# yangao07/LAMSA

Hardware: AMD Instinct MI355X
Metric: aligned Gbase/s, 10 kbp ONT-error reads (12%: sub/ins/del 4% each), -T ont2d vs GRCh37-sized stand-in; inputs resident in HBM when the timed region starts (upload excluded: see pcie_inclusive_*) (higher is better)
Workload: dtype int32

## Files before the change

### lamsa_amd/csrc/hp_align_api.hip

```cpp
#include <hip/hip_runtime.h>
#include <algorithm>
#include <atomic>
#include <map>
#include <mutex>
#include <stdlib.h>
#include <string.h>
#include <time.h>
#include "hp_phase.h"
#include "hp_handle.h"
#include "hp_hostprep.h"

using namespace hp;

#ifndef HP_WAVES_PER_SIMD
#define HP_WAVES_PER_SIMD 4
#endif
__global__ __launch_bounds__(64, HP_WAVES_PER_SIMD) void k_align_batch(AlignArgs a)
{
    __shared__ int32_t lds[HP_BOTH_LDS_WORDS];
    const int slot = blockIdx.x;
    for (;;) {
        int u = 0;
        if (wv::leader()) u = atomicAdd(a.counter, 1);
        u = wv::uni(u);
// ... 410 lines not shown
    S->valid = true;
    return LAMSA_HP_OK;
}

static int cap_waves(int n_waves, size_t slab_per_wave, int n_cu)
{
    static const size_t budget = []() { size_t f = 0, t = 0; if (hipMemGetInfo(&f, &t) != hipSuccess || t == 0) { t = (size_t)288 << 30; f = t; } return std::min(t / 4, f / 3); }();
    if (slab_per_wave * (size_t)n_waves <= budget) return n_waves;
    size_t fit = budget / (slab_per_wave ? slab_per_wave : 1);
    if (n_cu > 0 && fit >= (size_t)n_cu) fit -= fit % (size_t)n_cu;
    return fit < 1 ? 1 : (int)fit;
}

#ifdef HP_PROF
static void prof_report(Slot &T, const long long *d_prof, int n)
{
    if (!d_prof) return;
    {
        std::vector<long long> pr((size_t)n * 64);
        hipMemcpy(pr.data(), d_prof, sizeof(long long) * pr.size(), hipMemcpyDeviceToHost);
        if (const char *dump = getenv("LAMSA_HP_PROF_DUMP")) {
            if (FILE *fp = fopen(dump, "wb")) {
                for (int r = 0; r < n; ++r) { long long hl[2] = {T.h_H[r], T.h_len[r]}; fwrite(hl, 8, 2, fp); fwrite(&pr[(size_t)r * 64], 8, 64, fp); }
                fclose(fp);
            }
        }
        std::vector<int> idx((size_t)n); for (int i = 0; i < n; ++i) idx[i] = i;
        auto tot = [&](int r) { long long t = 0; for (int k = 0; k < 6; ++k) t += pr[(size_t)r * 64 + k]; return t; };
        std::sort(idx.begin(), idx.end(), [&](int x, int y) { return tot(x) > tot(y); });
        long long sum[64] = {0}; for (int r = 0; r < n; ++r) for (int k = 0; k < 64; ++k) sum[k] += pr[(size_t)r * 64 + k];
        fprintf(stderr, "[HP_PROF] cycles: setup chain1 fill1 chain2 fill2 publish | in chain1: init+minext mainscan track pop-loop bound+flines | o_l H\n");
        fprintf(stderr, "[HP_PROF] SUM  "); for (int k = 0; k < 11; ++k) fprintf(stderr, " %lld", sum[k] / 1000000); fprintf(stderr, " (Mcycles) targets %lld trips %lld init_Mcyc %lld\n", sum[11], sum[12], sum[13] / 1000000);
#ifdef HP_PROF_TRACK
        fprintf(stderr, "[HP_PROF] branch tracking (-DHP_PROF_TRACK: the line_build stamps below are off): marking pass %lld Mcyc; %lld seeds visited; %lld tracks, %lld Mcyc in them, %lld steps up; "
                        "%lld arrivals at a node with several sons, %lld Mcyc in cut_branch\n", sum[16] / 1000000, sum[19], sum[18], sum[17] / 1000000, sum[20], sum[21], sum[22] / 1000000);
#endif
        fprintf(stderr, "[HP_PROF] line_build: %lld lines (%lld without a gap), %lld anchors, %lld gaps | Mcyc: anchor walk %lld, gap list %lld, gaps in lanes %lld, gaps one by one %lld, assembly %lld\n",
                sum[21], sum[22], sum[12], sum[23], sum[16] / 1000000, sum[17] / 1000000, sum[18] / 1000000, sum[19] / 1000000, sum[20] / 1000000);
        fprintf(stderr, "[HP_PROF] gaps: %lld in lines with fewer than HP_GAP_MIN gaps (%lld lines with gaps); lane gaps: %lld hits scanned, %lld refused (range too long or too many active hits)\n", sum[54], sum[55], sum[11], sum[13]);
        { const char *nm[] = {"ksw_global", "ksw_extend", "backtrack", "ref_fetch", "head_fix", "frag_extend", "split_mapping", "tail_fix", "res_split", "res_aux", "mini_line_regs", "sort index"};
          for (int k = 0; k < 12; ++k) fprintf(stderr, "[HP_PROF] %-16s %8lld Mcyc %10lld calls\n", nm[k], sum[24 + 2 * k] / 1000000, sum[25 + 2 * k]);
#ifdef HP_PROF_FILL
          fprintf(stderr, "[HP_PROF] in frags_merge: boundary repair (merge_cigar_full) %lld Mcyc %lld calls; junctions through split_mapping %lld Mcyc %lld calls; fragments of several seeds %lld Mcyc %lld calls; 64-step gathers %lld Mcyc %lld\n", sum[16] / 1000000, sum[17], sum[18] / 1000000, sum[19], sum[20] / 1000000, sum[21], sum[22] / 1000000, sum[23]);
#endif
          fprintf(stderr, "[HP_PROF] direction-matrix bytes in HBM %lld (%lld jobs); hits passed through nodes_per_init %lld (%lld calls)\n", sum[52], sum[53], sum[54], sum[55]);
          fprintf(stderr, "[HP_PROF] chain_first start: seed loop %lld, node_set loop %lld, min_extend %lld Mcyc (%lld reads with a MIN pass)\n", sum[56] / 1000000, sum[57] / 1000000, sum[58] / 1000000, sum[59]);
          fprintf(stderr, "[HP_PROF] query <= 62: ksw_extend %lld Mcyc %lld calls, ksw_global %lld Mcyc %lld calls\n", sum[60] / 1000000, sum[61], sum[62] / 1000000, sum[63]);
          const char *bn[] = {"[bi_extend total]", "[bi_extend after left ext]", "17-32", "33-64", "65-128", "129-256", "257-512", ">512"};
          for (int k = 0; k < 2; ++k) fprintf(stderr, "[HP_PROF] ksw_extend qlen %-8s %8lld Mcyc %10lld calls\n", bn[k], sum[48 + 2 * k] / 1000000, sum[49 + 2 * k]); }
        {
            std::vector<long long> pd((size_t)n * 64);
            hipMemcpy(pd.data(), d_prof + ((size_t)n + 1) * 64, sizeof(long long) * pd.size(), hipMemcpyDeviceToHost);
            long long sd[64] = {0}; for (int r = 0; r < n; ++r) for (int k = 0; k < 64; ++k) sd[k] += pd[(size_t)r * 64 + k];
            const char *cn[] = {"one set, q <= 62", "packed, one set", "packed, two sets", "band 1 set", "band 2 sets", "band 4 sets", "int32 sets", "LDS / HBM rows"};
            for (int c = 0; c < 8; ++c) fprintf(stderr, "[HP_PROF] wave jobs, ksw_extend %-18s %8lld Mcyc %10lld Mcells %9lld calls %10lld rows\n", cn[c], sd[4 * c] / 1000000, sd[4 * c + 1] / 1000000, sd[4 * c + 2], sd[4 * c + 3]);
        }
        for (int q = 0; q < 8 && q < n; ++q) { int r = idx[q]; fprintf(stderr, "[HP_PROF] read %d L=%d:", r, T.h_len[r]); for (int k = 0; k < 11; ++k) fprintf(stderr, " %lld", pr[(size_t)r * 64 + k] / 1000000); fprintf(stderr, " | o_l %lld H %lld | targets %lld trips %lld init_Mcyc %lld\n", pr[(size_t)r * 64 + 14], pr[(size_t)r * 64 + 15], pr[(size_t)r * 64 + 11], pr[(size_t)r * 64 + 12], pr[(size_t)r * 64 + 13] / 1000000); }
    }
}
#endif

struct PhasedLayout { size_t bytes, o[15]; int unit_cap, lj_cap, wj_cap; int64_t fl_cap, line_cap, job_cap; };
static PhasedLayout phased_layout(int n, int64_t n_hits, int64_t n_bases, int64_t stream_cap)
{
    PhasedLayout Y;
    const size_t n_ent = (size_t)n_hits + (size_t)n + 1;
    Y.unit_cap = 8 * n + 1024;
    Y.fl_cap = 4 * n_hits + 2304 * (int64_t)n + 4096; Y.line_cap = stream_cap + 64 * (int64_t)Y.unit_cap;
    Y.job_cap = std::min<int64_t>(0x7fffff00ll, 4096 + 256 * (int64_t)n + 2 * n_bases);
    Y.lj_cap = (int)std::min<int64_t>(0x3fffffffll, 1024 + 16 * (int64_t)n + n_bases / 100);
    Y.wj_cap = (int)std::min<int64_t>(0x3fffffffll, 1024 + 32 * (int64_t)n + n_bases / 200);
    size_t off = 0;
    auto place = [&](size_t bytes) { size_t o = off; off = al256(off + bytes + 16); return o; };
    const size_t sz[15] = {sizeof(PhaseArgs), sizeof(PhaseCtl), sizeof(RdMeta) * ((size_t)n + 1), sizeof(NodeS) * n_ent, 4 * n_ent, 8 * n_ent, sizeof(UnitRec) * 2 * (size_t)Y.unit_cap,
                           4 * 2 * (size_t)PH_NBUCKET * Y.unit_cap, 4 * (size_t)Y.fl_cap, 4 * (size_t)Y.line_cap, 4 * (size_t)Y.job_cap, sizeof(LjRec) * (size_t)Y.lj_cap, 4 * (size_t)LJ_NBUCKET * Y.lj_cap,
                           sizeof(WjRec) * (size_t)Y.wj_cap, 4 * (size_t)WJ_NBUCKET * Y.wj_cap};
    for (int k = 0; k < 15; ++k) Y.o[k] = place(sz[k]);
    Y.bytes = off;
    return Y;
}
static int64_t main_stream_cap(int n, int64_t n_bases, int tags) { return 1024 + (int64_t)n * 256 + 4 * n_bases + (tags ? (int64_t)n * 128 + 2 * n_bases : 0); }

struct SlabPlan { size_t chain, fill, wj, wjb, wjb_off; int w_chain, w_fill, w_dp, w_wj, n_wjb, shape; size_t bytes; };
static int chain_shape(const lamsa_hp_para &P, int64_t n_reads, int64_t n_bases)
{
    static const int force = getenv("LAMSA_HP_CHAIN_SHAPE") ? atoi(getenv("LAMSA_HP_CHAIN_SHAPE")) : -1;
    if (force >= 0 && force < 3) return force;
    const int64_t mean_L = n_reads > 0 ? n_bases / n_reads : 0, ss = P.seed_step > 0 ? P.seed_step : 1;
    const int64_t est = mean_L / ss * 2 / 3;
    for (int k = 0; k < 2; ++k) if (est <= g_chain_shapes[k].lds_words / 5) return k;
    return 2;
}
static SlabPlan slab_plan(lamsa_hp_handle *h, int max_L, int max_H, bool shared = false, int shape = 0)
{
    SlabPlan Q;
    Q.shape = shape;
    const lamsa_hp_para &P = h->para;
    Q.chain = al256(((size_t)256 << 10) + 128 * (size_t)max_L + 424 * (size_t)max_H);
    Q.fill = al256(((size_t)256 << 10) + (h->result_tags ? 152 : 128) * (size_t)max_L + sizeof(cig_t) * 3 * HP_LJ_CIG * 64 + (size_t)HP_LJ_QSMALL * HP_LJ_TSMALL * 64 + 64);
    { static const int kb = getenv("LAMSA_HP_WJ_SLAB_KB") ? atoi(getenv("LAMSA_HP_WJ_SLAB_KB")) : 0;
      Q.wj = ((size_t)(kb > 0 ? kb : 1024) << 10) + 33 * 256; }
    Q.wjb = al256((size_t)wj_need(&P, WJ_HEAD, max_L, max_L + 2 * P.hash_step + 64) + ((size_t)64 << 10)) + 33 * 256;
    if (Q.wjb < Q.wj) Q.wjb = Q.wj;
    if (g_nowave) Q.fill = std::max(Q.fill, slab_bytes_for(P, max_L, max_H, 1, h->result_tags));
    if (h->scratch_limit) { const size_t lim = al256(h->scratch_limit); Q.chain = std::min(Q.chain, lim); Q.fill = std::min(Q.fill, lim); Q.wj = std::min(Q.wj, lim); Q.wjb = std::min(Q.wjb, lim); }
    int pc = 0, pf = 0, pd = 0, pw = 0;
    if (hipOccupancyMaxActiveBlocksPerMultiprocessor(&pc, g_chain_shapes[shape].k1, 64, 0) != hipSuccess || pc < 1) pc = 4 * g_chain_shapes[shape].waves_per_simd;
    if (hipOccupancyMaxActiveBlocksPerMultiprocessor(&pf, k_fill, 64, 0) != hipSuccess || pf < 1) pf = 4;
// ... 347 lines not shown
```

### lamsa_amd/csrc/hp_ksw.h

```cpp
#pragma once
#include "hp_core.h"

namespace hp {

#define HP_ZSTRIDE(n_col) ((((n_col) + 7) >> 3) << 2)
HP_INL size_t z_cap(const Ctx &cx) { const int w = cx.lds_words - (2 * HP_LDS_CELLS + HP_LDS_CELLS / 4); return w > 0 ? (size_t)w * 4 : 0; }
HP_INL size_t z_cap_pk(const Ctx &cx) { return cx.lds_words > 0 ? (size_t)cx.lds_words * 4 : 0; }
#define HP_ZFITS(n_col, rows) ((size_t)HP_ZSTRIDE(n_col) * (size_t)(rows) <= z_cap(cx))
HP_INL int z_nibble(int dir) { return (dir & 3) | ((dir >> 2) & 1) << 2 | ((dir >> 5) & 1) << 3; }
HP_INL void z_row_clear(HP_L uint8_t *LZ, int row, int n_col) {
    HP_L int *p = (HP_L int *)(LZ + row * HP_ZSTRIDE(n_col));
    const int nd = HP_ZSTRIDE(n_col) >> 2;
    for (int d0 = 0; d0 < nd; d0 += 64) { WAVE_FOR(l) { if (d0 + l < nd) p[d0 + l] = -1; } }
}
HP_INL void z_put(HP_L uint8_t *LZ, int row, int n_col, int c, int dir) {
    HP_L int *p = (HP_L int *)(LZ + row * HP_ZSTRIDE(n_col)) + (c >> 3);
    wv::lds_and(p, (int)~((unsigned)(~z_nibble(dir) & 0xf) << ((c & 7) << 2)));
}

HP_FN void dp_backtrack(Ctx &cx, const HP_L uint8_t *lz, const uint8_t *z, const int32_t *rowb, int n_col, int w, int i, int k, CigV &out, int pk_stride = 0)
{
    pk_stride = wv::uni(pk_stride);
    const bool in_lds = z == nullptr;
    const HP_G uint8_t *gz = (const HP_G uint8_t *)wv::uni64((long long)z);
// ... 763 lines not shown
                    if (j == end) Es[c][l] = 0;
                    nz[l] = j >= beg && j <= end && (Hs[c][l] != 0 || Es[c][l] != 0);
                }
                nzm[c] = wv::ballot(nz);
            }
            const int jj = beg < end ? end : beg;
            if (jj == qlen) {
                max_ie = gscore > h_last ? max_ie : i;
                gscore = gscore > h_last ? gscore : h_last;
            }
            if (mrow == 0) { stop_rows = true; break; }
            if (mrow > max) { max = mrow; max_i = i; max_j = mj; }
            else if (zdrop > 0) {
                if (i - max_i > mj - max_j) { if (max - mrow - ((i - max_i) - (mj - max_j)) * e_del > zdrop) { stop_rows = true; break; } }
                else { if (max - mrow - ((mj - max_j) - (i - max_i)) * e_ins > zdrop) { stop_rows = true; break; } }
            }
            {
                const int e_set = end >> 6;
                const unsigned long long e_bit = 1ull << (end & 63);
                bool end_nz = false, got = false;
                int nb = end, jl = -1;
#pragma unroll
                for (int c = 0; c < NS; ++c) {
                    unsigned long long lo = nzm[c];
                    if (c == e_set) { end_nz = lo & e_bit; lo &= ~e_bit; }
                    if (!got && lo) { nb = 64 * c + __builtin_ctzll(lo); got = true; }
                }
                if (got) {
                    bool gl = false;
#pragma unroll
                    for (int c = NS - 1; c >= 0; --c) if (!gl && nzm[c]) { jl = 64 * c + 63 - __builtin_clzll(nzm[c]); gl = true; }
                } else jl = end_nz ? end : end - 1;
                beg = nb;
                end = jl + 2 < qlen ? jl + 2 : qlen;
            }
        }
    }
    int i, k;
    if (gscore <= 0 || gscore <= max - end_bonus) { i = max_i; k = max_j; }
    else { i = max_ie; k = qlen - 1; }
    er.qle = k + 1; er.tle = i + 1; er.score = max;
    if (out) { wv::sync(); HP_T0(tb0_); dp_backtrack(cx, zl ? LZ : nullptr, z, rowb, n_col, w, i, k, *out); HP_TADD(cx, 28, tb0_); }
    cx.n_cells += cells_;
    arena_release(cx.tmp, mark);
    HP_TADD(cx, 26, te0_);
    return er;
}

#define HP_PK_QMAX(ns) (128 * (ns) - 2)
#ifndef HP_PK_RT
#define HP_PK_RT 1
#endif
#define HP_PK_IDENT (-16000)

HP_INL int pkb_sets_q(int qlen, int w)
{
    for (int ns = 1; ns <= 4; ns *= 2) if (2 * w + 3 + 18 * ns <= 128 * ns || qlen + 3 <= 128 * ns) return ns;
    return 0;
}
HP_INL bool pkb_extend_ok(const lamsa_hp_para *P, int qlen, int h0, int ns)
{
    const int mx = P->match > P->mis ? P->match : P->mis;
    const int pen = (P->ins_ext_o > P->del_ext_o ? P->ins_ext_o : P->del_ext_o) + (P->ins_ext_e > P->del_ext_e ? P->ins_ext_e : P->del_ext_e);
    const int ext = P->ins_ext_e > P->del_ext_e ? P->ins_ext_e : P->del_ext_e;
    return ns > 0 && mx > 0 && mx < 256 && pen >= 0 && pen < 4000 && P->ins_ext_e >= 0 && P->del_ext_e >= 0 && P->ins_ext_o >= 0 && P->del_ext_o >= 0 &&
           (long long)h0 + (long long)qlen * mx < 23000 && (long long)(128 * ns + 2) * ext < 8000 && qlen + 128 * ns < 32000;
}
template <int NS>
HP_NOINL ExtRes ksw_extend_band(Ctx &cx, int qlen, Seq q, int tlen, Seq t, int w, int h0, CigV *out)
{
    long long cells_ = 0;
    ExtRes er; er.score = 0; er.qle = 0; er.tle = 0;
    HP_T0(te0_);
    qlen = wv::uni(qlen); tlen = wv::uni(tlen); w = wv::uni(w); h0 = wv::uni(h0);
    const lamsa_hp_para *P = cx.P;
    const int o_ins = wv::uni(P->ins_ext_o), e_ins = wv::uni(P->ins_ext_e), o_del = wv::uni(P->del_ext_o), e_del = wv::uni(P->del_ext_e);
    const int end_bonus = wv::uni(P->end_bonus), zdrop = wv::uni(P->zdrop);
    const int oe_del = o_del + e_del, oe_ins = o_ins + e_ins;
    const int n_col = qlen < 2 * w + 1 ? qlen : 2 * w + 1;
    constexpr int LC = 2 * NS, WN = 128 * NS, zs = 64 * NS;
    const size_t mark = arena_mark(cx.tmp);
    uint8_t *z = (uint8_t *)arena_alloc(cx, (size_t)zs * tlen + 16);
    int32_t *rowb = (int32_t *)arena_alloc(cx, sizeof(int32_t) * 2 * ((size_t)tlen + 1));
    if (!z || !rowb) { arena_release(cx.tmp, mark); return er; }
#ifdef HP_PROF
    if (cx.prof) { cx.prof[52] += (long long)zs * tlen; cx.prof[53] += 1; }
#endif
    HP_G uint8_t *gz = (HP_G uint8_t *)wv::uni64((long long)z);
    HP_G int32_t *growb = (HP_G int32_t *)wv::uni64((long long)rowb);
    const int sc_match = wv::uni(P->match), sc_mis = -wv::uni(P->mis);
    const HP_G uint8_t *gq = (const HP_G uint8_t *)wv::uni64((long long)q.p); const int qs = wv::uni(q.stride);
    const HP_G uint8_t *gt = (const HP_G uint8_t *)wv::uni64((long long)t.p); const int ts = wv::uni(t.stride);
    const int h1v = h0 > oe_ins ? h0 - oe_ins : 0;
    const int OEI = pk::rep(oe_ins), OED = pk::rep(oe_del), EI = pk::rep(e_ins), ED = pk::rep(e_del);
    const int DSC = pk::rep(sc_match - sc_mis), MIS = pk::rep(sc_mis), IDENT = pk::rep(HP_PK_IDENT);
#define HP_PKB_EH0(j) ((j) == 0 ? h0 : ((j) == 1 ? h1v : (((j) <= qlen && h1v - ((j) - 2) * e_ins > e_ins) ? h1v - ((j) - 1) * e_ins : 0)))
#define HP_PKB_LOAD(jb_) do { \
        _Pragma("unroll") for (int r_ = 0; r_ < NS; ++r_) { \
            int hv_[2], oh_ = 0, nn_ = 0; \
            _Pragma("unroll") for (int b_ = 0; b_ < 2; ++b_) { \
                const int j_ = (jb_) + 2 * r_ + b_; \
                hv_[b_] = HP_PKB_EH0(j_); \
                const int code_ = j_ < qlen ? (int)gq[(long)j_ * qs] : 4; \
                if (code_ < 4) oh_ |= 1 << (code_ + 16 * b_); else nn_ |= (int)(0xffffu << (16 * b_)); \
            } \
            Hs[r_][l] = pk::pack(hv_[0], hv_[1]); Es[r_][l] = 0; qoh[r_][l] = oh_; qN[r_][l] = nn_; \
        } \
        JB[l] = pk::rep(jb_); } while (0)
    wv::Lane<int> Hs[NS], Es[NS], qoh[NS], qN[NS], hcur[NS], M[NS], INB[NS], JRE[NS], pre[NS], JB, tl;
    WAVE_FOR(l) { tl[l] = 4; HP_PKB_LOAD(LC * l); }
    int top = WN;
    int max = h0, max_i = -1, max_j = -1, max_ie = -1, gscore = -1;
    int beg = 0, end = qlen;
    bool stop_rows = false;
    for (int ib = 0; ib < tlen && !stop_rows; ib += 64) {
        { WAVE_FOR(l) { const int ii = ib + l; tl[l] = ii < tlen ? gt[(long)ii * ts] : 4; } }
        const int ti_first = wv::bcast(tl, 0);
        const int ie = ib + 64 < tlen ? ib + 64 : tlen;
        for (int i = ib; i < ie; ++i) {
            const int ti = i == ib ? ti_first : wv::bcast(tl, i & 63);
            if (beg < i - w) beg = i - w;
            if (end > i + w + 1) end = i + w + 1;
            if (end > qlen) end = qlen;
            cells_ += end > beg ? end - beg : 0;
            { WAVE_FOR(l) { if (l < 2) growb[2 * i + l] = l ? end : beg; } }
            int h1_init;
            if (beg == 0) { h1_init = h0 - (o_del + e_del * (i + 1)); if (h1_init < 0) h1_init = 0; }
            else h1_init = 0;
            if (beg >= end) {
                if (beg == qlen) { max_ie = gscore > h1_init ? max_ie : i; gscore = gscore > h1_init ? gscore : h1_init; }
                stop_rows = true; break;
            }
            if (end + 3 > top) {
                const int lr = (top / LC) & 63;
                WAVE_FOR(l) { const int d = (l - lr) & 63; if (d < 8) { const int jb = top + d * LC; HP_PKB_LOAD(jb); } }
                top += 8 * LC;
            }
            const int tsh = ti & 3, tN = ti > 3 ? -1 : 0;
            const int BEG = pk::rep(beg), END = pk::rep(end), H1 = pk::rep(h1_init);
            const int l0 = (beg / LC) & 63;
            wv::Lane<int> ka, kb;
            WAVE_FOR(l) {
                int run = HP_PK_IDENT;
#pragma unroll
                for (int r = 0; r < NS; ++r) {
                    const int jp = pk::add(JB[l], pk::pack(2 * r, 2 * r + 1));
                    const int in = pk::neg_mask(pk::sub(jp, END)) & ~pk::neg_mask(pk::sub(jp, BEG));
                    const int eq = (qoh[r][l] >> tsh) & 0x00010001;
                    const int S = pk::add(pk::mul(eq, DSC), MIS) | qN[r][l] | tN;
                    const int hm = Hs[r][l];
                    const int m = pk::mul(pk::add(hm, S), pk::min_u(hm, 0x00010001));
                    const int t1 = pk::max(pk::sub(m, OEI), 0);
                    const int jre = pk::mul(pk::sub(jp, BEG), EI);
                    const int k = pk::sel(in, pk::add(t1, jre), IDENT);
                    const int klo = pk::lo(k), khi = pk::hi(k);
                    const int p0 = run; run = run > klo ? run : klo;
                    const int p1 = run; run = run > khi ? run : khi;
                    M[r][l] = m; INB[r][l] = in; JRE[r][l] = jre; pre[r][l] = pk::pack(p0, p1);
                }
                ka[l] = l >= l0 ? run : HP_PK_IDENT; kb[l] = l < l0 ? run : HP_PK_IDENT;
            }
            const int topA = wv::scan_max_excl_top(ka, HP_PK_IDENT);
            wv::scan_max_excl(kb, HP_PK_IDENT);
            wv::Lane<int> best;
            WAVE_FOR(l) {
                const int pl = l >= l0 ? ka[l] : (topA > kb[l] ? topA : kb[l]);
                const int PP = pk::rep(pl);
                int zw = 0, bk = -1;
#pragma unroll
                for (int r = 0; r < NS; ++r) {
                    const int jre = JRE[r][l], in = INB[r][l], m = M[r][l];
                    const int pr = pk::max(pre[r][l], PP);
                    int f = pk::max(pk::add(pk::sub(pr, jre), EI), pk::sub(0, jre));
                    const int tI = pk::max(pk::sub(m, OEI), 0);
                    int ee = Es[r][l];
                    const int m1 = pk::neg_mask(pk::sub(ee, m));
                    int h = pk::max(m, ee);
                    const int m2 = pk::neg_mask(pk::sub(f, h));
                    int d = pk::sel(m2, ~m1 & 0x00010001, 0x00020002);
                    h = pk::max(h, f);
                    const int tD = pk::max(pk::sub(m, OED), 0);
                    ee = pk::sub(ee, ED);
                    d |= pk::neg_mask(pk::sub(tD, ee)) & 0x00040004;
                    ee = pk::max(ee, tD);
                    f = pk::sub(f, EI);
                    d |= pk::neg_mask(pk::sub(tI, f)) & 0x00080008;
                    Es[r][l] = pk::sel(in, ee, Es[r][l]);
                    const int hc = pk::sel(in, h, -1);
                    hcur[r][l] = hc;
                    zw |= ((d | (d >> 12)) & 0xff) << (8 * r);
                    const int jp = pk::add(JB[l], pk::pack(2 * r, 2 * r + 1));
                    const int k0 = (int)(((unsigned)hc << 16) | ((unsigned)jp & 0xffffu)), k1 = (int)(((unsigned)hc & 0xffff0000u) | ((unsigned)jp >> 16));
                    bk = bk > k0 ? bk : k0; bk = bk > k1 ? bk : k1;
                }
                best[l] = bk;
                if constexpr (NS == 1) gz[(long)i * zs + l] = (uint8_t)zw;
                else if constexpr (NS == 2) *(HP_G uint16_t *)(gz + (long)i * zs + 2 * l) = (uint16_t)zw;
                else *(HP_G uint32_t *)(gz + (long)i * zs + 4 * l) = (uint32_t)zw;
            }
            int mrow = 0, mj = -1;
            { const int b = wv::reduce_max(best); if (b >= 0) { mrow = b >> 16; mj = b & 0xffff; } }
            int h_last;
            {
                const int le = ((end - 1) / LC) & 63, sl = (end - 1) % LC;
                int v = 0;
#pragma unroll
                for (int r = 0; r < NS; ++r) if ((sl >> 1) == r) v = wv::bcast(hcur[r], le);
                h_last = (sl & 1) ? pk::hi(v) : pk::lo(v);
            }
            wv::Lane<int> rot = hcur[NS - 1], LB;
            wv::ror1(rot);
            WAVE_FOR(l) {
                int bits = 0;
#pragma unroll
                for (int r = 0; r < NS; ++r) {
                    const int below = r > 0 ? hcur[r > 0 ? r - 1 : 0][l] : rot[l];
                    const int hsh = pk::shift_up(hcur[r][l], below);
                    const int in = INB[r][l];
                    const int upd = ~pk::neg_mask(hsh);
                    int hs = Hs[r][l], es = Es[r][l];
                    hs = pk::sel(upd, hsh, hs);
                    hs = pk::sel(in & ~upd, H1, hs);
                    es &= ~(upd & ~in);
                    Hs[r][l] = hs; Es[r][l] = es;
                    const int nzh = pk::min_u((hs | es) & (in | upd), 0x00010001);
                    bits |= ((nzh | (nzh >> 15)) & 3) << (2 * r);
                }
                LB[l] = bits;
            }
            if (end == qlen) {
                max_ie = gscore > h_last ? max_ie : i;
                gscore = gscore > h_last ? gscore : h_last;
            }
            if (mrow == 0) { stop_rows = true; break; }
            if (mrow > max) { max = mrow; max_i = i; max_j = mj; }
            else if (zdrop > 0) {
                if (i - max_i > mj - max_j) { if (max - mrow - ((i - max_i) - (mj - max_j)) * e_del > zdrop) { stop_rows = true; break; } }
                else { if (max - mrow - ((mj - max_j) - (i - max_i)) * e_ins > zdrop) { stop_rows = true; break; } }
            }
            {
                const unsigned long long any = wv::ballot(LB);
                int nb = end, jl = end - 1;
                if (any) {
                    const unsigned long long rt = l0 ? ((any >> l0) | (any << (64 - l0))) : any;
                    const int df = __builtin_ctzll(rt), dl = 63 - __builtin_clzll(rt);
                    const int bf = wv::bcast(LB, (l0 + df) & 63), bl = wv::bcast(LB, (l0 + dl) & 63);
                    const int bb = beg / LC;
                    const int jf = (bb + df) * LC + __builtin_ctz((unsigned)bf), jx = (bb + dl) * LC + (31 - __builtin_clz((unsigned)bl));
                    if (jf < end) nb = jf;
                    jl = jx;
                }
                beg = nb;
                end = jl + 2 < qlen ? jl + 2 : qlen;
            }
        }
    }
#undef HP_PKB_LOAD
#undef HP_PKB_EH0
    int i, k;
    if (gscore <= 0 || gscore <= max - end_bonus) { i = max_i; k = max_j; }
    else { i = max_ie; k = qlen - 1; }
    er.qle = k + 1; er.tle = i + 1; er.score = max;
    if (out) { wv::sync(); HP_T0(tb0_); dp_backtrack(cx, nullptr, z, rowb, n_col, w, i, k, *out, zs); HP_TADD(cx, 28, tb0_); }
    cx.n_cells += cells_;
    arena_release(cx.tmp, mark);
    HP_TADD(cx, 26, te0_);
    return er;
}

#define HP_PKG_NEG (-12000)
#define HP_PKG_IDENT (-24000)
HP_INL bool pk_global_ok(const lamsa_hp_para *P, int qlen, int tlen, int o_del, int e_del, int o_ins, int e_ins)
{
    const int mx = P->match > P->mis ? P->match : P->mis;
    const long long o = o_del > o_ins ? o_del : o_ins, e = e_del > e_ins ? e_del : e_ins;
    return mx > 0 && mx < 256 && o_del >= 0 && e_del >= 0 && o_ins >= 0 && e_ins >= 0 && o + e * ((long long)qlen + tlen + 4) + (long long)mx * (qlen + 2) < 4000;
}
template <int NS>
HP_NOINL int ksw_global_pk(Ctx &cx, int qlen, Seq q, int tlen, Seq t, int o_del, int e_del, int o_ins, int e_ins, int w, CigV *out)
{
    long long cells_ = 0;
    HP_T0(tg0_);
    qlen = wv::uni(qlen); tlen = wv::uni(tlen); w = wv::uni(w);
    o_del = wv::uni(o_del); e_del = wv::uni(e_del); o_ins = wv::uni(o_ins); e_ins = wv::uni(e_ins);
    const int oe_del = o_del + e_del, oe_ins = o_ins + e_ins;
    const int n_col = qlen < 2 * w + 1 ? qlen : 2 * w + 1;
    const int zs = 64 * NS;
    const size_t mark = arena_mark(cx.tmp);
    const bool zl = (size_t)zs * (size_t)tlen <= z_cap_pk(cx);
    if (out && zl) ++cx.lds_epoch;
    uint8_t *z = (out && !zl) ? (uint8_t *)arena_alloc(cx, (size_t)zs * tlen + 1) : nullptr;
    if (out && !zl && !z) { arena_release(cx.tmp, mark); return 0; }
    HP_L uint8_t *LZ = (HP_L uint8_t *)cx.lds;
    HP_G uint8_t *gz = (HP_G uint8_t *)wv::uni64((long long)z);
    const int sc_match = wv::uni(cx.P->match), sc_mis = -wv::uni(cx.P->mis);
    const HP_G uint8_t *gq = (const HP_G uint8_t *)wv::uni64((long long)q.p); const int qs = wv::uni(q.stride);
    const HP_G uint8_t *gt = (const HP_G uint8_t *)wv::uni64((long long)t.p); const int ts = wv::uni(t.stride);
    const int OEI = pk::rep(oe_ins), OED = pk::rep(oe_del), EI = pk::rep(e_ins), ED = pk::rep(e_del);
    const int DSC = pk::rep(sc_match - sc_mis), MIS = pk::rep(sc_mis), IDENT = pk::rep(HP_PKG_IDENT), NEG = pk::rep(HP_PKG_NEG);
    wv::Lane<int> Hs[NS], Es[NS], qoh[NS], qN[NS], hcur[NS], jp0, jep0, tl;
    WAVE_FOR(l) { jp0[l] = pk::pack(2 * l, 2 * l + 1); jep0[l] = pk::pack(2 * l * e_ins, (2 * l + 1) * e_ins); tl[l] = 4; }
#pragma unroll
    for (int c = 0; c < NS; ++c) {
        WAVE_FOR(l) {
            int hv[2], oh = 0, nn = 0;
#pragma unroll
            for (int b = 0; b < 2; ++b) {
                const int j = 128 * c + 2 * l + b;
                hv[b] = j == 0 ? 0 : (j <= w ? -(o_ins + e_ins * j) : HP_PKG_NEG);
                const int code = j < qlen ? (int)gq[(long)j * qs] : 4;
                if (code < 4) oh |= 1 << (code + 16 * b); else nn |= (int)(0xffffu << (16 * b));
            }
            Hs[c][l] = pk::pack(hv[0], hv[1]); Es[c][l] = NEG;
            qoh[c][l] = oh; qN[c][l] = nn;
        }
    }
// ... 239 lines not shown
        if (mrow > max) { max = mrow; max_i = i; max_j = mj; }
        else if (zdrop > 0) {
            if (i - max_i > mj - max_j) { if (max - mrow - ((i - max_i) - (mj - max_j)) * e_del > zdrop) { stop_rows = true; break; } }
            else { if (max - mrow - ((mj - max_j) - (i - max_i)) * e_ins > zdrop) { stop_rows = true; break; } }
        }
        {
            const int nb = first_nz >= 0 ? first_nz : end;
            int jl;
            if (h_last != 0 && end >= nb) jl = end;
            else if (last_nz >= nb && last_nz >= 0) jl = last_nz;
            else jl = nb - 1;
            beg = nb;
            end = jl + 2 < qlen ? jl + 2 : qlen;
        }
    }
    }
#undef HP_EH0
    int i, k;
    if (gscore <= 0 || gscore <= max - end_bonus) { i = max_i; k = max_j; }
    else { i = max_ie; k = qlen - 1; }
    er.qle = k + 1; er.tle = i + 1; er.score = max;
    if (out) { wv::sync(); HP_T0(tb0_); dp_backtrack(cx, zl ? LZ : nullptr, z, rowb, n_col, w, i, k, *out); HP_TADD(cx, 28, tb0_); }
    cx.n_cells += cells_;
    arena_release(cx.tmp, mark);
    HP_TADD(cx, 26, te0_);
    return er;
}

HP_INL int ksw_extend(Ctx &cx, int qlen, Seq q, int tlen, Seq t, int w, int h0, int *qle, int *tle, CigV *out)
{
    if (out) out->n = 0;
    if (qle) *qle = 0;
    if (tle) *tle = 0;
    if (qlen < 0 || tlen < 0 || h0 <= 0) { cx.status |= ST_REFEXIT; return 0; }
    {
        const lamsa_hp_para *P = cx.P;
        int mx = P->match > 0 ? P->match : 0;
        if (-P->mis > mx) mx = -P->mis;
        int max_ins = (int)((double)(qlen * mx + P->end_bonus - P->ins_ext_o) / P->ins_ext_e + 1.);
        max_ins = max_ins > 1 ? max_ins : 1;
        w = w < max_ins ? w : max_ins;
        int max_del = (int)((double)(qlen * mx + P->end_bonus - P->del_ext_o) / P->del_ext_e + 1.);
        max_del = max_del > 1 ? max_del : 1;
        w = w < max_del ? w : max_del;
    }
    const long long cells0_ = cx.n_cells; (void)cells0_;
    ExtRes er;
    int cls_ = 0; (void)cls_;
    HP_T0(tcls_);
    if (qlen <= HP_REG_QMAX) er = ksw_extend_reg(cx, qlen, q, tlen, t, w, h0, out);
    else if (HP_PK_RT && pkb_extend_ok(cx.P, qlen, h0, pkb_sets_q(qlen, w))) {
        HP_STAT(22);
        const int ns = pkb_sets_q(qlen, w);
        cls_ = ns == 1 ? 3 : (ns == 2 ? 4 : 5);
        er = ns == 1 ? ksw_extend_band<1>(cx, qlen, q, tlen, t, w, h0, out) : (ns == 2 ? ksw_extend_band<2>(cx, qlen, q, tlen, t, w, h0, out) : ksw_extend_band<4>(cx, qlen, q, tlen, t, w, h0, out));
    }
    else if (qlen <= HP_REGN_QMAX(2)) { HP_STAT(17); cls_ = 6; er = ksw_extend_regn<2>(cx, qlen, q, tlen, t, w, h0, out); }
    else if (qlen <= HP_REGN_QMAX(3) && HP_REGN_SETS >= 3) { HP_STAT(17); cls_ = 6; er = ksw_extend_regn<3>(cx, qlen, q, tlen, t, w, h0, out); }
    else if (qlen <= HP_REGN_QMAX(4) && HP_REGN_SETS >= 4) { HP_STAT(17); cls_ = 6; er = ksw_extend_regn<4>(cx, qlen, q, tlen, t, w, h0, out); }
    else { cls_ = 7; er = 2 * w + 4 + 64 <= HP_LDS_CELLS ? ksw_extend_lds(cx, qlen, q, tlen, t, w, h0, out) : ksw_extend_wide(cx, qlen, q, tlen, t, w, h0, out); }
#ifdef HP_PROF
    if (cx.prof_dp) { cx.prof_dp[4 * cls_] += wv::clock() - tcls_; cx.prof_dp[4 * cls_ + 1] += cx.n_cells - cells0_; cx.prof_dp[4 * cls_ + 2] += 1; cx.prof_dp[4 * cls_ + 3] += er.tle; }
#endif
    HP_DPLOG(0, qlen, tlen, w, cx.n_cells - cells0_);
    if (qle) *qle = er.qle;
    if (tle) *tle = er.tle;
    return er.score;
}

HP_INL int ksw_extend_c(Ctx &cx, int qlen, Seq q, int tlen, Seq t, int w, int h0, int *qle, int *tle, CigV *out)
{
    ksw_extend(cx, qlen, q, tlen, t, w, h0, qle, tle, out);
    if (*qle == qlen) return 0;
    if (*tle == tlen) return 1;
    return 2;
}
HP_INL int ksw_extend_r(Ctx &cx, int qlen, Seq q, int tlen, Seq t, int w, int h0, int *qre, int *tre, CigV *out)
{
    Seq rq, rt;
    rq.p = q.p + (long)(qlen > 0 ? qlen - 1 : 0) * q.stride; rq.stride = -q.stride;
    rt.p = t.p + (long)(tlen > 0 ? tlen - 1 : 0) * t.stride; rt.stride = -t.stride;
    ksw_extend(cx, qlen, rq, tlen, rt, w, h0, qre, tre, out);
    if (*qre == qlen) return 0;
    if (*tre == tlen) return 1;
    return 2;
}

HP_INL void sw_mid_fix(Ctx &cx, CigV &out, const cig_t *lc, int ln, const cig_t *rc, int rn,
                      int qlen, Seq q, int lqe, int rqe, int tlen, Seq t, int lte, int rte)
{
    const lamsa_hp_para *P = cx.P;
    int Sn = qlen - lqe - rqe, Hn = tlen - lte - rte, half = P->split_len / 2;
    if (iabs(Sn) >= half || iabs(Hn) >= half || iabs(Sn - Hn) >= half || tlen < 0 || qlen < 0) {
        cig_pushv(cx, out, lc, ln);
        cig_push0(cx, out, (cig_t)((uint32_t)Sn << 4) | C_S);
        cig_push0(cx, out, (cig_t)((uint32_t)Hn << 4) | C_H);
        cig_pushv(cx, out, rc, rn);
    } else {
        const size_t mark = arena_mark(cx.tmp);
        CigV g;
        if (cig_alloc(cx, g, qlen + tlen + 2)) {
            ksw_global(cx, qlen, q, tlen, t, P->del_gapo, P->del_gape, P->ins_gapo, P->ins_gape, P->band_w, &g);
            cig_pushv(cx, out, g.c, g.n);
        }
        arena_release(cx.tmp, mark);
    }
}

HP_INL bool bi_near_diag(const lamsa_hp_para *P, int qlen, int tlen)
{
#if defined(__HIP_DEVICE_COMPILE__)
    float a = __fmul_rn((float)tlen, P->id_rate);
    float b = __fmul_rn(a, (float)(P->aln_mode & 2));
    float c = __fadd_rn((float)P->split_len, b);
#else
    volatile float a = (float)tlen * P->id_rate;
    volatile float b = a * (float)(P->aln_mode & 2);
    volatile float c = (float)P->split_len + b;
#endif
    return (float)iabs(qlen - tlen) < c;
}

HP_NOINL int ksw_bi_extend(Ctx &cx_, int qlen, Seq q, int tlen, Seq t, int lh0, int rh0, CigV &out_)
{
    HP_STAT(31);
    Ctx &cx = *(Ctx *)wv::uni64((long long)&cx_);
    CigV &out = *(CigV *)wv::uni64((long long)&out_);
    qlen = wv::uni(qlen); tlen = wv::uni(tlen); lh0 = wv::uni(lh0); rh0 = wv::uni(rh0);
    q.p = (const uint8_t *)wv::uni64((long long)q.p); q.stride = wv::uni(q.stride);
    t.p = (const uint8_t *)wv::uni64((long long)t.p); t.stride = wv::uni(t.stride);
    const lamsa_hp_para *P = (const lamsa_hp_para *)wv::uni64((long long)cx.P);
    out.n = 0;
    if (qlen < 0 || tlen < 0) { cx.status |= ST_REFEXIT; return 0; }
    if (qlen == 0 && lh0 > 0) {
        if (tlen > 0) cig_raw_push(cx, out, (tlen << 4) | C_D);
        return 0;
    }
    HP_T0(tbi0_);
    const size_t mark = arena_mark(cx.tmp);
    int ret = 0, res, lqe, lte, rqe, rte;
    CigV L, R;
    if (!cig_alloc(cx, L, qlen + tlen + 4) || !cig_alloc(cx, R, qlen + tlen + 4)) { arena_release(cx.tmp, mark); return 0; }
    L.c = (cig_t *)wv::uni64((long long)L.c); R.c = (cig_t *)wv::uni64((long long)R.c); L.cap = wv::uni(L.cap); R.cap = wv::uni(R.cap);
    const int band_w = wv::uni(P->band_w);
    const int w = iabs(qlen - tlen) + 3 > band_w ? iabs(qlen - tlen) + 3 : band_w;
    res = ksw_extend_c(cx, qlen, q, tlen, t, w, lh0, &lqe, &lte, &L);
    res = wv::uni(res); lqe = wv::uni(lqe); lte = wv::uni(lte);
    HP_T0(tbi1_);
    if (res < 2) {
        cig_pushv(cx, out, L.c, L.n);
        cig_push1(cx, out, res == 0 ? ((tlen - lte) << 4) | C_D : ((qlen - lqe) << 4) | C_I);
    } else if (bi_near_diag(P, qlen, tlen) && ((lqe << 1 > qlen) || (lte << 1 > tlen))) {
        ksw_global(cx, qlen, q, tlen, t, P->del_gapo, P->del_gape, P->ins_gapo, P->ins_gape, P->band_w, &out);
    } else {
        res = ksw_extend_r(cx, qlen, q, tlen, t, w, rh0, &rqe, &rte, &R);
        res = wv::uni(res); rqe = wv::uni(rqe); rte = wv::uni(rte);
        if (res < 2) {
            cig_push1(cx, R, res == 0 ? ((tlen - rte) << 4) | C_D : ((qlen - rqe) << 4) | C_I);
            cig_invert(R.c, R.n);
            cig_pushv(cx, out, R.c, R.n);
        } else if (bi_near_diag(P, qlen, tlen) && ((rqe << 1 > qlen) || (rte << 1 > tlen))) {
            ksw_global(cx, qlen, q, tlen, t, P->del_gapo, P->del_gape, P->ins_gapo, P->ins_gape, P->band_w, &out);
        } else {
            cig_invert(R.c, R.n);
            sw_mid_fix(cx, out, L.c, L.n, R.c, R.n, qlen, q, lqe, rqe, tlen, t, lte, rte);
            ret = (qlen - lqe - rqe) >= P->split_len ? 1 : 0;
        }
    }
    arena_release(cx.tmp, mark);
    HP_TADD(cx, 50, tbi1_);
    HP_TADD(cx, 48, tbi0_);
    return ret;
}

}
```

### lamsa_amd/csrc/hp_wavejob.h

```cpp
#pragma once
#include "hp_lanedp.h"

namespace hp {

enum { WJ_BI = 1, WJ_GLOBAL = 2, WJ_HEAD = 3, WJ_TAIL = 4 };
struct WjRec { int64_t qaddr, tk, slot; int32_t rd, qlen, tlen, type_comp; };
enum { WJ_NBIG = 4, WJ_NSMALL = 12, WJ_NBUCKET = WJ_NBIG + WJ_NSMALL };

HP_HD long long wj_need(const lamsa_hp_para *P, int type, int qlen, int tlen)
{
    const int d = qlen > tlen ? qlen - tlen : tlen - qlen;
    const int w = type == WJ_BI && d + 3 > P->band_w ? d + 3 : P->band_w;
    long long ncol = qlen < 2 * w + 1 ? qlen : 2 * w + 1;
    if (ncol < 256) ncol = 256;
    return ((long long)64 << 10) + 40ll * ((long long)qlen + tlen) + 16ll * qlen + ncol * ((long long)tlen + 16);
}

HP_INL int wj_bucket_of(const lamsa_hp_para *P, int type, int qlen, int tlen, bool big)
{
    const int band = 2 * P->band_w + 1, cols = qlen < band ? qlen : band;
    const long long cost = (long long)(type == WJ_HEAD || type == WJ_TAIL ? qlen : tlen) * (cols > 0 ? cols : 1);
    int b = 0;
    if (big) { for (long long c = cost >> 20; c > 0 && b < WJ_NBIG - 1; c >>= 1) ++b; return WJ_NBIG - 1 - b; }
    for (long long c = cost >> 11; c > 0 && b < WJ_NSMALL - 1; c >>= 1) ++b;
    return WJ_NBIG + WJ_NSMALL - 1 - b;
}

#ifndef HP_WJ_WAVES_PER_SIMD
#define HP_WJ_WAVES_PER_SIMD 8
#endif
#ifndef HP_WJ_LDS_WORDS
#define HP_WJ_LDS_WORDS HP_LDS_WORDS
#endif

struct WjOut { int score, qle, tle, reflen, readlen; };

HP_FN bool wj_run(Ctx &cx, const uint8_t *reads, const uint8_t *pac, int type, int comp, int64_t qaddr, int qs, int qlen, int64_t tk, int ts, int tlen,
                  int w, int h0, CigV &out, WjOut &o)
{
    const lamsa_hp_para *P = cx.P;
    o.score = 0; o.qle = 0; o.tle = 0; o.reflen = 0; o.readlen = 0;
    out.n = 0;
    uint8_t *qb = (uint8_t *)arena_alloc(cx, (size_t)(qlen > 0 ? qlen : 0) + 16), *tb = (uint8_t *)arena_alloc(cx, (size_t)(tlen > 0 ? tlen : 0) + 16);
    if (!qb || !tb) return false;
    {
        const HP_G uint8_t *gr = (const HP_G uint8_t *)reads + qaddr, *gp = (const HP_G uint8_t *)pac;
        HP_G uint8_t *gq = (HP_G uint8_t *)qb, *gt = (HP_G uint8_t *)tb;
        for (int b = 0; b < qlen; b += 64) { WAVE_FOR(l) { const int j = b + l; if (j < qlen) { const int c = gr[(long)j * qs]; gq[j] = (uint8_t)(comp ? (c < 4 ? 3 - c : 4) : c); } } }
        for (int b = 0; b < tlen; b += 64) { WAVE_FOR(l) { const int i = b + l; if (i < tlen) { const int64_t k = tk + (int64_t)i * ts; gt[i] = (uint8_t)(gp[k >> 2] >> ((~k & 3) << 1) & 3); } } }
        wv::sync();
    }
    const Seq q = seq_fwd(qb), t = seq_fwd(tb);
    if (type == WJ_BI) o.score = ksw_bi_extend(cx, qlen, q, tlen, t, h0, h0, out);
    else if (type == WJ_GLOBAL) o.score = ksw_global(cx, qlen, q, tlen, t, P->del_gapo, P->del_gape, P->ins_gapo, P->ins_gape, w, &out);
    else {
        o.score = ksw_extend(cx, qlen, q, tlen, t, w, h0, &o.qle, &o.tle, &out);
        const int rr = o.qle == qlen ? 0 : (o.tle == tlen ? 1 : 2);
        if (rr != 0) cig_push1(cx, out, ((qlen - o.qle) << 4) | C_S);
        if (type == WJ_HEAD) cig_invert(out.c, out.n);
    }
    wv::sync();
    if (cx.status & (ST_REFEXIT | ST_OVERFLOW)) return false;
    o.reflen = cig_reflen(out.c, out.n); o.readlen = cig_readlen(out.c, out.n);
    return true;
}

}
```

Before: 3.943.

## Add fixed-window specialization of packed banded ksw_extend when query fits in lanes

Adds a FIXED template variant of ksw_extend_band used when the whole query fits in the wave's packed columns. This variant skips the sliding-window reload, the rotated two-part prefix-max scan and the per-row lane offset math. It also precomputes the per-column gap term once, moves the last-column broadcast under the end==qlen branch, and builds keys with a byte-permute intrinsic. Profiling counters for the new class are added under HP_PROF. The risk is that the precomputed gap term relative to beg (the F0 offset) changes numeric results if it is not exactly equivalent.

```diff
diff --git a/lamsa_amd/csrc/hp_align_api.hip b/lamsa_amd/csrc/hp_align_api.hip
--- a/lamsa_amd/csrc/hp_align_api.hip
+++ b/lamsa_amd/csrc/hp_align_api.hip
@@ -486,8 +486,12 @@
             std::vector<long long> pd((size_t)n * 64);
             hipMemcpy(pd.data(), d_prof + ((size_t)n + 1) * 64, sizeof(long long) * pd.size(), hipMemcpyDeviceToHost);
             long long sd[64] = {0}; for (int r = 0; r < n; ++r) for (int k = 0; k < 64; ++k) sd[k] += pd[(size_t)r * 64 + k];
-            const char *cn[] = {"one set, q <= 62", "packed, one set", "packed, two sets", "band 1 set", "band 2 sets", "band 4 sets", "int32 sets", "LDS / HBM rows"};
-            for (int c = 0; c < 8; ++c) fprintf(stderr, "[HP_PROF] wave jobs, ksw_extend %-18s %8lld Mcyc %10lld Mcells %9lld calls %10lld rows\n", cn[c], sd[4 * c] / 1000000, sd[4 * c + 1] / 1000000, sd[4 * c + 2], sd[4 * c + 3]);
+            const char *cn[] = {"one set, q <= 62", "packed, one set", "packed, two sets", "band 1 set slides", "band 2 sets slides", "band 4 sets slides", "int32 sets", "LDS / HBM rows",
+                                "band 1 set fixed", "band 2 sets fixed", "band 4 sets fixed"};
+            for (int c = 0; c < 11; ++c) fprintf(stderr, "[HP_PROF] wave jobs, ksw_extend %-18s %8lld Mcyc %10lld Mcells %9lld calls %10lld rows\n", cn[c], sd[4 * c] / 1000000, sd[4 * c + 1] / 1000000, sd[4 * c + 2], sd[4 * c + 3]);
+            fprintf(stderr, "[HP_PROF] wave jobs, junctions of the class 'band 2 sets fixed': %lld jobs, wj_run %lld Mcyc of which staging %lld; ksw_bi_extend %lld Mcyc of which after the left extension %lld; "
+                            "in ksw_extend_band<2>: setup and first fill %lld, rows %lld, backtrack %lld Mcyc\n",
+                    sd[51], sd[50] / 1000000, sd[49] / 1000000, sd[47] / 1000000, sd[48] / 1000000, sd[44] / 1000000, sd[45] / 1000000, sd[46] / 1000000);
         }
         for (int q = 0; q < 8 && q < n; ++q) { int r = idx[q]; fprintf(stderr, "[HP_PROF] read %d L=%d:", r, T.h_len[r]); for (int k = 0; k < 11; ++k) fprintf(stderr, " %lld", pr[(size_t)r * 64 + k] / 1000000); fprintf(stderr, " | o_l %lld H %lld | targets %lld trips %lld init_Mcyc %lld\n", pr[(size_t)r * 64 + 14], pr[(size_t)r * 64 + 15], pr[(size_t)r * 64 + 11], pr[(size_t)r * 64 + 12], pr[(size_t)r * 64 + 13] / 1000000); }
     }
diff --git a/lamsa_amd/csrc/hp_ksw.h b/lamsa_amd/csrc/hp_ksw.h
--- a/lamsa_amd/csrc/hp_ksw.h
+++ b/lamsa_amd/csrc/hp_ksw.h
@@ -839,6 +839,14 @@
 #define HP_PK_RT 1
 #endif
 #define HP_PK_IDENT (-16000)
+#ifdef HP_PROF
+#define HP_PD2_T0(v) const long long v = wv::clock()
+#define HP_PD2_ADD(cx, on, slot, v) do { if ((cx).prof_dp && (on)) (cx).prof_dp[slot] += wv::clock() - (v); } while (0)
+#define HP_PD2_CLASS(qlen, w) (pkb_sets_q(qlen, w) == 2 && (qlen) + 3 <= 256)
+#else
+#define HP_PD2_T0(v) do { } while (0)
+#define HP_PD2_ADD(cx, on, slot, v) do { } while (0)
+#endif
 
 HP_INL int pkb_sets_q(int qlen, int w)
 {
@@ -853,18 +861,36 @@
     return ns > 0 && mx > 0 && mx < 256 && pen >= 0 && pen < 4000 && P->ins_ext_e >= 0 && P->del_ext_e >= 0 && P->ins_ext_o >= 0 && P->del_ext_o >= 0 &&
            (long long)h0 + (long long)qlen * mx < 23000 && (long long)(128 * ns + 2) * ext < 8000 && qlen + 128 * ns < 32000;
 }
-template <int NS>
+HP_INL int pkb_key_lo(int h, int j)
+{
+#if defined(__HIP_DEVICE_COMPILE__)
+    return (int)__builtin_amdgcn_perm((unsigned)h, (unsigned)j, 0x05040100u);
+#else
+    return (int)(((unsigned)h << 16) | ((unsigned)j & 0xffffu));
+#endif
+}
+HP_INL int pkb_key_hi(int h, int j)
+{
+#if defined(__HIP_DEVICE_COMPILE__)
+    return (int)__builtin_amdgcn_perm((unsigned)h, (unsigned)j, 0x07060302u);
+#else
+    return (int)(((unsigned)h & 0xffff0000u) | ((unsigned)j >> 16));
+#endif
+}
+template <int NS, bool FIXED>
 HP_NOINL ExtRes ksw_extend_band(Ctx &cx, int qlen, Seq q, int tlen, Seq t, int w, int h0, CigV *out)
 {
     long long cells_ = 0;
     ExtRes er; er.score = 0; er.qle = 0; er.tle = 0;
     HP_T0(te0_);
     qlen = wv::uni(qlen); tlen = wv::uni(tlen); w = wv::uni(w); h0 = wv::uni(h0);
+    HP_PD2_T0(tp0_);
     const lamsa_hp_para *P = cx.P;
     const int o_ins = wv::uni(P->ins_ext_o), e_ins = wv::uni(P->ins_ext_e), o_del = wv::uni(P->del_ext_o), e_del = wv::uni(P->del_ext_e);
     const int end_bonus = wv::uni(P->end_bonus), zdrop = wv::uni(P->zdrop);
     const int oe_del = o_del + e_del, oe_ins = o_ins + e_ins;
     const int n_col = qlen < 2 * w + 1 ? qlen : 2 * w + 1;
+    constexpr bool KEY0 = FIXED && NS < 4, KEEP_JRE = NS < 4;
     constexpr int LC = 2 * NS, WN = 128 * NS, zs = 64 * NS;
     const size_t mark = arena_mark(cx.tmp);
     uint8_t *z = (uint8_t *)arena_alloc(cx, (size_t)zs * tlen + 16);
@@ -893,13 +919,22 @@
             } \
             Hs[r_][l] = pk::pack(hv_[0], hv_[1]); Es[r_][l] = 0; qoh[r_][l] = oh_; qN[r_][l] = nn_; \
         } \
-        JB[l] = pk::rep(jb_); } while (0)
+        JB[l] = pk::pack(jb_, (jb_) + 1); } while (0)
     wv::Lane<int> Hs[NS], Es[NS], qoh[NS], qN[NS], hcur[NS], M[NS], INB[NS], JRE[NS], pre[NS], JB, tl;
     WAVE_FOR(l) { tl[l] = 4; HP_PKB_LOAD(LC * l); }
-    int top = WN;
+    if constexpr (FIXED) HP_STAT(16);
+    if constexpr (KEY0) {
+        WAVE_FOR(l) {
+#pragma unroll
+            for (int r = 0; r < NS; ++r) JRE[r][l] = pk::mul(pk::add(JB[l], pk::rep(2 * r)), EI);
+        }
+    }
+    int top = WN; (void)top;
     int max = h0, max_i = -1, max_j = -1, max_ie = -1, gscore = -1;
     int beg = 0, end = qlen;
     bool stop_rows = false;
+    HP_PD2_ADD(cx, NS == 2 && qlen + 3 <= WN, 44, tp0_);
+    HP_PD2_T0(tp1_);
     for (int ib = 0; ib < tlen && !stop_rows; ib += 64) {
         { WAVE_FOR(l) { const int ii = ib + l; tl[l] = ii < tlen ? gt[(long)ii * ts] : 4; } }
         const int ti_first = wv::bcast(tl, 0);
@@ -918,47 +953,52 @@
                 if (beg == qlen) { max_ie = gscore > h1_init ? max_ie : i; gscore = gscore > h1_init ? gscore : h1_init; }
                 stop_rows = true; break;
             }
-            if (end + 3 > top) {
+            if (!FIXED && end + 3 > top) {
                 const int lr = (top / LC) & 63;
                 WAVE_FOR(l) { const int d = (l - lr) & 63; if (d < 8) { const int jb = top + d * LC; HP_PKB_LOAD(jb); } }
                 top += 8 * LC;
             }
             const int tsh = ti & 3, tN = ti > 3 ? -1 : 0;
             const int BEG = pk::rep(beg), END = pk::rep(end), H1 = pk::rep(h1_init);
-            const int l0 = (beg / LC) & 63;
+            const int l0 = FIXED ? 0 : (beg / LC) & 63;
+            const int F0 = KEY0 ? pk::rep(beg * e_ins) : 0;
             wv::Lane<int> ka, kb;
             WAVE_FOR(l) {
                 int run = HP_PK_IDENT;
 #pragma unroll
                 for (int r = 0; r < NS; ++r) {
-                    const int jp = pk::add(JB[l], pk::pack(2 * r, 2 * r + 1));
+                    const int jp = pk::add(JB[l], pk::rep(2 * r));
                     const int in = pk::neg_mask(pk::sub(jp, END)) & ~pk::neg_mask(pk::sub(jp, BEG));
                     const int eq = (qoh[r][l] >> tsh) & 0x00010001;
                     const int S = pk::add(pk::mul(eq, DSC), MIS) | qN[r][l] | tN;
                     const int hm = Hs[r][l];
                     const int m = pk::mul(pk::add(hm, S), pk::min_u(hm, 0x00010001));
                     const int t1 = pk::max(pk::sub(m, OEI), 0);
-                    const int jre = pk::mul(pk::sub(jp, BEG), EI);
+                    const int jre = KEY0 ? JRE[r][l] : pk::mul(pk::sub(jp, BEG), EI);
                     const int k = pk::sel(in, pk::add(t1, jre), IDENT);
                     const int klo = pk::lo(k), khi = pk::hi(k);
                     const int p0 = run; run = run > klo ? run : klo;
                     const int p1 = run; run = run > khi ? run : khi;
-                    M[r][l] = m; INB[r][l] = in; JRE[r][l] = jre; pre[r][l] = pk::pack(p0, p1);
-                }
-                ka[l] = l >= l0 ? run : HP_PK_IDENT; kb[l] = l < l0 ? run : HP_PK_IDENT;
-            }
-            const int topA = wv::scan_max_excl_top(ka, HP_PK_IDENT);
-            wv::scan_max_excl(kb, HP_PK_IDENT);
+                    M[r][l] = m; INB[r][l] = in; if constexpr (!KEY0 && KEEP_JRE) JRE[r][l] = jre; pre[r][l] = pk::pack(p0, p1);
+                }
+                if constexpr (FIXED) { ka[l] = run; kb[l] = HP_PK_IDENT; }
+                else { ka[l] = l >= l0 ? run : HP_PK_IDENT; kb[l] = l < l0 ? run : HP_PK_IDENT; }
+            }
+            int topA = HP_PK_IDENT;
+            if constexpr (FIXED) wv::scan_max_excl(ka, HP_PK_IDENT);
+            else { topA = wv::scan_max_excl_top(ka, HP_PK_IDENT); wv::scan_max_excl(kb, HP_PK_IDENT); }
             wv::Lane<int> best;
             WAVE_FOR(l) {
-                const int pl = l >= l0 ? ka[l] : (topA > kb[l] ? topA : kb[l]);
+                const int pl = FIXED ? ka[l] : (l >= l0 ? ka[l] : (topA > kb[l] ? topA : kb[l]));
                 const int PP = pk::rep(pl);
                 int zw = 0, bk = -1;
 #pragma unroll
                 for (int r = 0; r < NS; ++r) {
-                    const int jre = JRE[r][l], in = INB[r][l], m = M[r][l];
+                    const int jp = pk::add(JB[l], pk::rep(2 * r));
+                    const int jre = KEEP_JRE ? JRE[r][l] : pk::mul(pk::sub(jp, BEG), EI);
+                    const int in = INB[r][l], m = M[r][l];
                     const int pr = pk::max(pre[r][l], PP);
-                    int f = pk::max(pk::add(pk::sub(pr, jre), EI), pk::sub(0, jre));
+                    int f = pk::max(pk::add(pk::sub(pr, jre), EI), pk::sub(F0, jre));
                     const int tI = pk::max(pk::sub(m, OEI), 0);
                     int ee = Es[r][l];
                     const int m1 = pk::neg_mask(pk::sub(ee, m));
@@ -976,8 +1016,7 @@
                     const int hc = pk::sel(in, h, -1);
                     hcur[r][l] = hc;
                     zw |= ((d | (d >> 12)) & 0xff) << (8 * r);
-                    const int jp = pk::add(JB[l], pk::pack(2 * r, 2 * r + 1));
-                    const int k0 = (int)(((unsigned)hc << 16) | ((unsigned)jp & 0xffffu)), k1 = (int)(((unsigned)hc & 0xffff0000u) | ((unsigned)jp >> 16));
+                    const int k0 = pkb_key_lo(hc, jp), k1 = pkb_key_hi(hc, jp);
                     bk = bk > k0 ? bk : k0; bk = bk > k1 ? bk : k1;
                 }
                 best[l] = bk;
@@ -987,14 +1026,6 @@
             }
             int mrow = 0, mj = -1;
             { const int b = wv::reduce_max(best); if (b >= 0) { mrow = b >> 16; mj = b & 0xffff; } }
-            int h_last;
-            {
-                const int le = ((end - 1) / LC) & 63, sl = (end - 1) % LC;
-                int v = 0;
-#pragma unroll
-                for (int r = 0; r < NS; ++r) if ((sl >> 1) == r) v = wv::bcast(hcur[r], le);
-                h_last = (sl & 1) ? pk::hi(v) : pk::lo(v);
-            }
             wv::Lane<int> rot = hcur[NS - 1], LB;
             wv::ror1(rot);
             WAVE_FOR(l) {
@@ -1016,6 +1047,11 @@
                 LB[l] = bits;
             }
             if (end == qlen) {
+                const int le = FIXED ? (end - 1) / LC : ((end - 1) / LC) & 63, sl = (end - 1) % LC;
+                int v = 0;
+#pragma unroll
+                for (int r = 0; r < NS; ++r) if ((sl >> 1) == r) v = wv::bcast(hcur[r], le);
+                const int h_last = (sl & 1) ? pk::hi(v) : pk::lo(v);
                 max_ie = gscore > h_last ? max_ie : i;
                 gscore = gscore > h_last ? gscore : h_last;
             }
@@ -1031,8 +1067,8 @@
                 if (any) {
                     const unsigned long long rt = l0 ? ((any >> l0) | (any << (64 - l0))) : any;
                     const int df = __builtin_ctzll(rt), dl = 63 - __builtin_clzll(rt);
-                    const int bf = wv::bcast(LB, (l0 + df) & 63), bl = wv::bcast(LB, (l0 + dl) & 63);
-                    const int bb = beg / LC;
+                    const int bf = wv::bcast(LB, FIXED ? df : (l0 + df) & 63), bl = wv::bcast(LB, FIXED ? dl : (l0 + dl) & 63);
+                    const int bb = FIXED ? 0 : beg / LC;
                     const int jf = (bb + df) * LC + __builtin_ctz((unsigned)bf), jx = (bb + dl) * LC + (31 - __builtin_clz((unsigned)bl));
                     if (jf < end) nb = jf;
                     jl = jx;
@@ -1048,7 +1084,10 @@
     if (gscore <= 0 || gscore <= max - end_bonus) { i = max_i; k = max_j; }
     else { i = max_ie; k = qlen - 1; }
     er.qle = k + 1; er.tle = i + 1; er.score = max;
+    HP_PD2_ADD(cx, NS == 2 && qlen + 3 <= WN, 45, tp1_);
+    HP_PD2_T0(tp2_);
     if (out) { wv::sync(); HP_T0(tb0_); dp_backtrack(cx, nullptr, z, rowb, n_col, w, i, k, *out, zs); HP_TADD(cx, 28, tb0_); }
+    HP_PD2_ADD(cx, NS == 2 && qlen + 3 <= WN, 46, tp2_);
     cx.n_cells += cells_;
     arena_release(cx.tmp, mark);
     HP_TADD(cx, 26, te0_);
@@ -1394,8 +1433,11 @@
     else if (HP_PK_RT && pkb_extend_ok(cx.P, qlen, h0, pkb_sets_q(qlen, w))) {
         HP_STAT(22);
         const int ns = pkb_sets_q(qlen, w);
-        cls_ = ns == 1 ? 3 : (ns == 2 ? 4 : 5);
-        er = ns == 1 ? ksw_extend_band<1>(cx, qlen, q, tlen, t, w, h0, out) : (ns == 2 ? ksw_extend_band<2>(cx, qlen, q, tlen, t, w, h0, out) : ksw_extend_band<4>(cx, qlen, q, tlen, t, w, h0, out));
+        cls_ = (ns == 1 ? 3 : (ns == 2 ? 4 : 5)) + (qlen + 3 <= 128 * ns ? 5 : 0);
+        if (qlen + 3 <= 128 * ns)
+            er = ns == 1 ? ksw_extend_band<1, true>(cx, qlen, q, tlen, t, w, h0, out) : (ns == 2 ? ksw_extend_band<2, true>(cx, qlen, q, tlen, t, w, h0, out) : ksw_extend_band<4, true>(cx, qlen, q, tlen, t, w, h0, out));
+        else
+            er = ns == 1 ? ksw_extend_band<1, false>(cx, qlen, q, tlen, t, w, h0, out) : (ns == 2 ? ksw_extend_band<2, false>(cx, qlen, q, tlen, t, w, h0, out) : ksw_extend_band<4, false>(cx, qlen, q, tlen, t, w, h0, out));
     }
     else if (qlen <= HP_REGN_QMAX(2)) { HP_STAT(17); cls_ = 6; er = ksw_extend_regn<2>(cx, qlen, q, tlen, t, w, h0, out); }
     else if (qlen <= HP_REGN_QMAX(3) && HP_REGN_SETS >= 3) { HP_STAT(17); cls_ = 6; er = ksw_extend_regn<3>(cx, qlen, q, tlen, t, w, h0, out); }
@@ -1479,6 +1521,7 @@
         return 0;
     }
     HP_T0(tbi0_);
+    HP_PD2_T0(tpb0_);
     const size_t mark = arena_mark(cx.tmp);
     int ret = 0, res, lqe, lte, rqe, rte;
     CigV L, R;
@@ -1489,6 +1532,7 @@
     res = ksw_extend_c(cx, qlen, q, tlen, t, w, lh0, &lqe, &lte, &L);
     res = wv::uni(res); lqe = wv::uni(lqe); lte = wv::uni(lte);
     HP_T0(tbi1_);
+    HP_PD2_T0(tpb1_);
     if (res < 2) {
         cig_pushv(cx, out, L.c, L.n);
         cig_push1(cx, out, res == 0 ? ((tlen - lte) << 4) | C_D : ((qlen - lqe) << 4) | C_I);
@@ -1510,6 +1554,8 @@
         }
     }
     arena_release(cx.tmp, mark);
+    HP_PD2_ADD(cx, HP_PD2_CLASS(qlen, w), 47, tpb0_);
+    HP_PD2_ADD(cx, HP_PD2_CLASS(qlen, w), 48, tpb1_);
     HP_TADD(cx, 50, tbi1_);
     HP_TADD(cx, 48, tbi0_);
     return ret;
diff --git a/lamsa_amd/csrc/hp_wavejob.h b/lamsa_amd/csrc/hp_wavejob.h
--- a/lamsa_amd/csrc/hp_wavejob.h
+++ b/lamsa_amd/csrc/hp_wavejob.h
@@ -41,6 +41,7 @@
     const lamsa_hp_para *P = cx.P;
     o.score = 0; o.qle = 0; o.tle = 0; o.reflen = 0; o.readlen = 0;
     out.n = 0;
+    HP_PD2_T0(tpw0_);
     uint8_t *qb = (uint8_t *)arena_alloc(cx, (size_t)(qlen > 0 ? qlen : 0) + 16), *tb = (uint8_t *)arena_alloc(cx, (size_t)(tlen > 0 ? tlen : 0) + 16);
     if (!qb || !tb) return false;
     {
@@ -50,6 +51,12 @@
         for (int b = 0; b < tlen; b += 64) { WAVE_FOR(l) { const int i = b + l; if (i < tlen) { const int64_t k = tk + (int64_t)i * ts; gt[i] = (uint8_t)(gp[k >> 2] >> ((~k & 3) << 1) & 3); } } }
         wv::sync();
     }
+#ifdef HP_PROF
+    const int wcls_ = iabs(qlen - tlen) + 3 > P->band_w ? iabs(qlen - tlen) + 3 : P->band_w;
+    const bool pcls_ = type == WJ_BI && HP_PD2_CLASS(qlen, wcls_);
+    if (cx.prof_dp && pcls_) cx.prof_dp[51] += 1;
+#endif
+    HP_PD2_ADD(cx, pcls_, 49, tpw0_);
     const Seq q = seq_fwd(qb), t = seq_fwd(tb);
     if (type == WJ_BI) o.score = ksw_bi_extend(cx, qlen, q, tlen, t, h0, h0, out);
     else if (type == WJ_GLOBAL) o.score = ksw_global(cx, qlen, q, tlen, t, P->del_gapo, P->del_gape, P->ins_gapo, P->ins_gape, w, &out);
@@ -60,6 +67,7 @@
         if (type == WJ_HEAD) cig_invert(out.c, out.n);
     }
     wv::sync();
+    HP_PD2_ADD(cx, pcls_, 50, tpw0_);
     if (cx.status & (ST_REFEXIT | ST_OVERFLOW)) return false;
     o.reflen = cig_reflen(out.c, out.n); o.readlen = cig_readlen(out.c, out.n);
     return true;
```

Result: faster. 4.030 (median of 6 runs) (+2.2%).
